# isaac-sim/IsaacGymEnvs

Measured on AMD Instinct MI355X. Metric: env-steps/sec (num_envs x control-steps/sec), random-action rollout, higher is better.
Workload: dtype f32; 1 GPU; Ant num_envs=4096 per GPU (4096 total), VecTask.step() via Python API, actions = 2*torch.rand-1 drawn before every step (README.md:48-51), seed 42+rank; 11000 untimed settle steps (about 0.5 s of back-to-back stepping at the BASELINE size) precede the 5 warm-ups; task=Ant, num_envs_per_gpu=4096, parallelism=env-shard x1, multi_wave=16, fused_sub=1, fused_post=1

## Files before the change

### isaacgymenvs_amd/csrc/core/engine_mw.hpp

```cpp
#pragma once
#include "engine.hpp"

namespace mi {

template <class M>
struct SimMW : Sim<M> {
    using B = Sim<M>;
    using typename B::Ctx;
    using typename B::BodyTmp;
    static constexpr int NB = B::NB, ND = B::ND, NV = B::NV, OFF = B::OFF, NSPH = B::NSPH, NSENS = B::NSENS, NLIM = B::NLIM,
                         NROWG = B::NROWG, NVA = B::NVA, NR = M::NROLE;

    static constexpr int role_of_body(int b) { return M::role_of_limb[M::limb_of_body[b]]; }
    static constexpr int role_of_gi(int gi) { return gi < OFF ? -1 : role_of_body(M::dof_body[gi - OFF]); }
    static constexpr bool trunk_body(int b) { return role_of_body(b) < 0; }
    static constexpr bool trunk_gi(int gi) { return role_of_gi(gi) < 0; }
    template <int R> static constexpr bool owns_body(int b) { return role_of_body(b) == R || (trunk_body(b) && R == M::TRUNK_ROLE); }
    template <int R> static constexpr bool owns_gi(int gi) { return role_of_gi(gi) == R || (trunk_gi(gi) && R == M::TRUNK_ROLE); }
    template <int R> static constexpr bool sees_gi(int gi) { return role_of_gi(gi) == R || trunk_gi(gi); }
    static constexpr int NTB = []() constexpr { int n = 0; for (int b = 0; b < NB; ++b) n += trunk_body(b) ? 1 : 0; return n; }();
    static constexpr int tslot(int b) { int n = 0; for (int k = 0; k < b; ++k) n += trunk_body(k) ? 1 : 0; return n; }
    static constexpr int NVT = []() constexpr { int n = 0; for (int i = 0; i < NV; ++i) n += trunk_gi(i) ? 1 : 0; return n; }();
    static constexpr int tidx(int gi) { int n = 0; for (int k = 0; k < gi; ++k) n += trunk_gi(k) ? 1 : 0; return n; }
    static constexpr int entry_row(int e) {
        for (int i = 0; i < NV; ++i)
            for (int j = 0; j <= i; ++j)
                if (M::midx[i][j] == e) return i;
        return 0;
    }
    static constexpr bool trunk_entry(int e) { return trunk_gi(entry_row(e)); }
    static constexpr int NTE = []() constexpr { int n = 0; for (int e = 0; e < M::NM; ++e) n += trunk_entry(e) ? 1 : 0; return n; }();
    static constexpr int teidx(int e) { int n = 0; for (int k = 0; k < e; ++k) n += trunk_entry(k) ? 1 : 0; return n; }
    static constexpr bool limb_root(int b) { return b > 0 && !trunk_body(b) && trunk_body(M::parent[b]); }
    static constexpr int NLR = []() constexpr { int n = 0; for (int b = 0; b < NB; ++b) n += limb_root(b) ? 1 : 0; return n; }();
    static constexpr int lridx(int b) { int n = 0; for (int k = 0; k < b; ++k) n += limb_root(k) ? 1 : 0; return n; }
    static constexpr int X_LR = B::ROW_SLOTS_STATIC;
    static constexpr int X_DT = X_LR + 16 * NLR;
    static constexpr int X_DY = X_DT + NR * NTE;
    static constexpr int X_DW = X_DY + NR * NVT;
    static constexpr int X_FLG = X_DW + 2 * NR * NVT;
    static constexpr int X_AT = X_FLG + 2 * NR;
    static constexpr int MW_SLOTS = X_AT + NROWG;

    static constexpr int NUNIT = NLIM + NSPH;
    template <int R> static constexpr bool own_unit(int u) {
        if (u < 0 || u >= NUNIT) return false;
        return u < NLIM ? owns_gi<R>(OFF + B::limdof(u)) : owns_body<R>(M::sph_body[u - NLIM]);
    }
    template <int R> static constexpr int next_own(int u) {
        for (int k = u + 1; k < NUNIT; ++k) if (own_unit<R>(k)) return k;
        return NUNIT;
    }
    template <int R> static constexpr int own_pos(int u) { int n = 0; for (int k = 0; k < u; ++k) n += own_unit<R>(k) ? 1 : 0; return n; }

    template <int R, int b, int XLR, int RS>
    MI_HD void trunk_down(const SimParams& P, Ctx& c, BodyTmp (&tb)[NTB], const float* Rp, const float* rp, const float* Vp,
                          const float* Ap, const RowStore<RS> rows) {
        constexpr int ts = tslot(b);
        BodyTmp& t = tb[ts];
        this->template body_down<b>(P, c, Rp, rp, Vp, Ap, t);
        sfor<NB>([&](auto C_) MI_LAMBDA {
            constexpr int ch = C_;
            if constexpr (ch > b) if constexpr (M::parent[ch] == b) {
                if constexpr (trunk_body(ch)) {
                    trunk_down<R, ch, XLR>(P, c, tb, t.Rb, t.rb, t.Vc, t.Ac, rows);
                } else if constexpr (role_of_body(ch) == R) {
                    SpI Ic;
                    float Fc[6];
                    this->template body_pass<ch>(P, c, t.Rb, t.rb, t.Vc, t.Ac, Ic, Fc);
                    constexpr int o = XLR + 16 * lridx(ch);
                    rows(o) = Ic.m;
                    sfor<3>([&](auto K) MI_LAMBDA { rows(o + 1 + K) = Ic.h[K]; });
                    sfor<6>([&](auto K) MI_LAMBDA { rows(o + 4 + K) = Ic.I[K]; rows(o + 10 + K) = Fc[K]; });
                }
            }
        });
    }

    float sens_own[6 * M::NSENSA];
    template <int R, bool KEEP = false, bool SENS = false, int RS, class GND, class BAR>
    MI_HD void substep_role(const SimParams& P, const float* tau, const float h, const RowStore<RS> rows, const Strided lamc,
                            const Strided laml, const Strided sensor, const Strided dof_force, const GND& gnd, const float mu_env,
                            const Strided netf, const int stage, const BAR& bar) {
        static_assert(!M::FIXED, "multi-wave sub-step: free-base models");
        auto G = [&](int row, int cc) MI_LAMBDA -> float& { return rows(row * M::MAXCHAIN + cc); };
        auto Ainv = [&](int row) MI_LAMBDA -> float& { return rows(NROWG * M::MAXCHAIN + row); };
        auto vt = [&](int row) MI_LAMBDA -> float& { return rows(NROWG * M::MAXCHAIN + NROWG + row); };
        auto lam = [&](int row) MI_LAMBDA -> float& { return rows(NROWG * M::MAXCHAIN + 2 * NROWG + row); };
        const float invh = MI_RCP(h);
        float (&root)[13] = this->root;
        float (&q)[M::NDA] = this->q;
        float (&qd)[M::NDA] = this->qd;
#if defined(MI_TIMING)
        unsigned long long* const tstamp = this->tstamp;
#endif
        MI_STAMP(0);
        Ctx c;
        float (&S)[M::NDA][6] = c.S;
        float (&L)[M::NM] = c.L;
        if (stage == 0) {
            sfor<ND>([&](auto D) MI_LAMBDA {
                constexpr int d = D;
                if constexpr (M::dof_limited[d] && owns_gi<R>(OFF + d)) { constexpr int o = B::stage_slot_lim(d); rows(o) = laml(d); }
            });
            sfor<3 * NSPH>([&](auto K) MI_LAMBDA {
                if constexpr (owns_body<R>(M::sph_body[K / 3])) { constexpr int o = B::stage_slot_con(K); rows(o) = lamc(K); }
            });
        }
        BodyTmp tb[NTB];
        static_assert(!B::COMPACT && B::LAM_IN_ROWS, "substep_role: models on the static row store");
        trunk_down<R, 0, X_LR>(P, c, tb, nullptr, nullptr, nullptr, nullptr, rows);
        MI_PHASE();
        float Ldi[NVA], y[NVA], w[NVA], v[NVA];
        v[0] = root[7]; v[1] = root[8]; v[2] = root[9]; v[3] = root[10]; v[4] = root[11]; v[5] = root[12];
        sfor<ND>([&](auto D) MI_LAMBDA { v[OFF + D] = qd[D]; });
        sfor<M::NM>([&](auto E_) MI_LAMBDA { if constexpr (trunk_entry(E_)) L[E_] = 0.f; });
        sfor<NV>([&](auto I) MI_LAMBDA { if constexpr (trunk_gi(I)) y[I] = 0.f; });
        float sc_damp[M::NDA], sc_stiff[M::NDA], sc_arm[M::NDA];
        sfor<ND>([&](auto D) MI_LAMBDA { sc_damp[D] = 1.f; sc_stiff[D] = 1.f; sc_arm[D] = 1.f; });
        if constexpr (B::SCALED) {
            if (this->actor_scale.p != nullptr) {
                sfor<ND>([&](auto D) MI_LAMBDA {
                    if constexpr (sees_gi<R>(OFF + D)) {
                        sc_damp[D] = this->actor_scale(B::AS_DAMP + D); sc_stiff[D] = this->actor_scale(B::AS_STIFF + D); sc_arm[D] = this->actor_scale(B::AS_ARM + D);
                    }
                });
            }
        }
        sfor<ND>([&](auto D) MI_LAMBDA {
            constexpr int d = D, gi = OFF + d;
            if constexpr (role_of_gi(gi) == R) {
                const float K = M::dof_stiffness[d] * sc_stiff[d], Dm = M::dof_damping[d] * sc_damp[d];
                L[M::midx[gi][gi]] += M::dof_armature[d] * sc_arm[d] + h * Dm + h * h * K;
                y[gi] = tau[d] - c.bias[gi] - K * (q[d] - M::dof_springref[d]) - (Dm + h * K) * qd[d];
            }
        });
        auto factor = [&](auto K_) MI_LAMBDA {
            constexpr int k = decltype(K_)::value;
            const float dk2 = fmaxf(L[M::midx[k][k]], 1e-30f);
            const float inv = MI_RSQ(dk2);
            L[M::midx[k][k]] = dk2 * inv;
            Ldi[k] = inv;
            sfor<M::nanc[k]>([&](auto A_) MI_LAMBDA { L[M::midx[k][M::anc[k][A_]]] *= inv; });
            sfor<M::nanc[k]>([&](auto A_) MI_LAMBDA {
                constexpr int i = M::anc[k][A_];
                const float lki = L[M::midx[k][i]];
                L[M::midx[i][i]] -= lki * lki;
                sfor<M::nanc[i]>([&](auto B_) MI_LAMBDA {
                    constexpr int j = M::anc[i][B_];
                    L[M::midx[i][j]] -= lki * L[M::midx[k][j]];
                });
            });
        };
        auto whiten = [&](auto I_) MI_LAMBDA {
            constexpr int i = decltype(I_)::value;
            const float z = y[i] * Ldi[i];
            sfor<M::nanc[i]>([&](auto A_) MI_LAMBDA { y[M::anc[i][A_]] -= L[M::midx[i][M::anc[i][A_]]] * z; });
            float s = L[M::midx[i][i]] * v[i];
            sfor<M::nanc[i]>([&](auto A_) MI_LAMBDA { s += L[M::midx[i][M::anc[i][A_]]] * v[M::anc[i][A_]]; });
            w[i] = s + h * z;
        };
        sfor_rev<NV>([&](auto K_) MI_LAMBDA { if constexpr (role_of_gi(K_) == R) factor(K_); });
        MI_PHASE();
        sfor_rev<NV>([&](auto I_) MI_LAMBDA { if constexpr (role_of_gi(I_) == R) whiten(I_); });
        sfor<M::NM>([&](auto E_) MI_LAMBDA { if constexpr (trunk_entry(E_)) { constexpr int o = X_DT + R * NTE + teidx(E_); rows(o) = L[E_]; } });
        sfor<NV>([&](auto I) MI_LAMBDA { if constexpr (trunk_gi(I)) { constexpr int o = X_DY + R * NVT + tidx(I); rows(o) = y[I]; } });
// ... 220 lines not shown
                        Bf.vt = rit(NROWG * M::MAXCHAIN + NROWG + row0);
                    }
                };
                auto unit_on = [&](auto U_) MI_LAMBDA -> bool {
                    constexpr int u = decltype(U_)::value;
                    if constexpr (u < NLIM) return true;
                    else if constexpr (u < NUNIT) return (sph_active >> (u - NLIM) & 1ull) != 0ull;
                    else return false;
                };
                constexpr int U0 = next_own<R>(-1);
                if constexpr (U0 < NUNIT) load_unit(std::integral_constant<int, U0>{}, ub[0]);
                sfor<NUNIT>([&](auto U_) MI_LAMBDA {
                    constexpr int u = U_;
                    if constexpr (own_unit<R>(u)) {
                        constexpr int pos = own_pos<R>(u), un = next_own<R>(u);
                        UBuf& Bf = ub[pos & 1];
                        if (unit_on(std::integral_constant<int, un>{}))
                            load_unit(std::integral_constant<int, un>{}, ub[(pos + 1) & 1]);
                        MI_PHASE();
                        if (!unit_on(std::integral_constant<int, u>{})) return;
                        if constexpr (u < NLIM) {
                            constexpr int d = B::limdof(u), gi = OFF + d, row = u;
                            float vn = Bf.g[0][0] * wget(std::integral_constant<int, gi>{});
                            sfor<M::nanc[gi]>([&](auto A_) MI_LAMBDA { vn += Bf.g[0][1 + A_] * wget(std::integral_constant<int, M::anc[gi][A_]>{}); });
                            const float lo = Bf.lam[0];
                            const float nl = fmaxf(lo - (vn - Bf.vt) * MI_RCP(Bf.al[0] + om * Bf.at[0]), 0.f);
                            const float dl = nl - lo;
                            lam(row) = nl;
                            actn = (nl > 0.f) ? 1.f : actn;
                            wupd(std::integral_constant<int, gi>{}, Bf.g[0][0] * dl);
                            sfor<M::nanc[gi]>([&](auto A_) MI_LAMBDA { wupd(std::integral_constant<int, M::anc[gi][A_]>{}, Bf.g[0][1 + A_] * dl); });
                        } else {
                            constexpr int s = u - NLIM, b = M::sph_body[s], row0 = NLIM + 3 * s;
                            const float mu = 0.5f * ((mu_env >= 0.f ? mu_env : M::sph_mu[s]) + P.plane_mu);
                            float ainv[3];
                            sfor<3>([&](auto K) MI_LAMBDA { ainv[K] = MI_RCP(Bf.al[K] + om * Bf.at[K]); });
                            float ln;
                            {
                                float vn = 0.f;
                                sfor<M::chain_len[b]>([&](auto C) MI_LAMBDA { vn += Bf.g[0][C] * wget(std::integral_constant<int, M::chain[b][C]>{}); });
                                const float lo = Bf.lam[0];
                                ln = fmaxf(lo - (vn - Bf.vt) * ainv[0], 0.f);
                                const float dl = ln - lo;
                                lam(row0) = ln;
                                actn = (ln > 0.f) ? 1.f : actn;
                                sfor<M::chain_len[b]>([&](auto C) MI_LAMBDA { wupd(std::integral_constant<int, M::chain[b][C]>{}, Bf.g[0][C] * dl); });
                            }
                            float lt[2], vtg[2];
                            sfor<2>([&](auto K) MI_LAMBDA {
                                float vn = 0.f;
                                sfor<M::chain_len[b]>([&](auto C) MI_LAMBDA { vn += Bf.g[1 + K][C] * wget(std::integral_constant<int, M::chain[b][C]>{}); });
                                vtg[K] = vn;
                                lt[K] = Bf.lam[1 + K] - vn * ainv[1 + K];
                            });
                            friction_disc(lt, Bf.lam[1], Bf.lam[2], vtg[0], vtg[1], ainv[1], ainv[2], mu * ln);
                            sfor<2>([&](auto K) MI_LAMBDA {
                                constexpr int row = row0 + 1 + K;
                                const float nl = lt[K], dl = nl - Bf.lam[1 + K];
                                lam(row) = nl;
                                sfor<M::chain_len[b]>([&](auto C) MI_LAMBDA { wupd(std::integral_constant<int, M::chain[b][C]>{}, Bf.g[1 + K][C] * dl); });
                            });
                        }
                    }
                });
                sfor<NV>([&](auto I) MI_LAMBDA { if constexpr (trunk_gi(I)) { constexpr int ti = tidx(I); xout(R * NVT + ti) = (wtl[ti] - w[I]) * iom; } });
                fout(R) = actn;
                bar();
                sfor<NV>([&](auto I) MI_LAMBDA {
                    constexpr int i = I;
                    if constexpr (trunk_gi(i)) { sfor<NR>([&](auto R_) MI_LAMBDA { constexpr int o = R_ * NVT + tidx(i); w[i] += xout(o); }); }
                });
            }
        }
        MI_STAMP(5);
        sfor<NV>([&](auto I_) MI_LAMBDA {
            constexpr int i = I_;
            if constexpr (sees_gi<R>(i)) {
                float s = w[i];
                sfor<M::nanc[i]>([&](auto A_) MI_LAMBDA { s -= L[M::midx[i][M::anc[i][A_]]] * v[M::anc[i][A_]]; });
                v[i] = s * Ldi[i];
            }
        });
        MI_PHASE();
        sfor<ND>([&](auto D) MI_LAMBDA {
            constexpr int d = D;
            if constexpr (owns_gi<R>(OFF + d)) {
                float ll = 0.f;
                if constexpr (M::dof_limited[d]) {
                    constexpr int row = B::limrow(d);
                    const float dl = q[d] - this->template limit_lower<d>(), du = this->template limit_upper<d>() - q[d];
                    ll = (dl < du) ? lam(row) : -lam(row);
                    if constexpr (KEEP) lam(row) = ll;
                }
                laml(d) = ll;
                dof_force(d) = tau[d] - M::dof_stiffness[d] * sc_stiff[d] * (q[d] - M::dof_springref[d]) - M::dof_damping[d] * sc_damp[d] * v[OFF + d] + ll * invh;
            }
        });
        float sens[6 * M::NSENSA];
        sfor<6 * NSENS>([&](auto K) MI_LAMBDA { sens[K] = 0.f; });
        float nf[GND::NETF ? NB : 1][3];
        if constexpr (GND::NETF) sfor<NB>([&](auto B_) MI_LAMBDA { nf[B_][0] = nf[B_][1] = nf[B_][2] = 0.f; });
        sfor<NSPH>([&](auto S_) MI_LAMBDA {
            constexpr int s = S_, b = M::sph_body[s], row0 = NLIM + 3 * s;
            if constexpr (owns_body<R>(b)) {
                if (!(sph_active >> s & 1ull)) {
                    lamc(3 * s) = 0.f; lamc(3 * s + 1) = 0.f; lamc(3 * s + 2) = 0.f;
                    return;
                }
                const float ln = lam(row0), l1 = lam(row0 + 1), l2 = lam(row0 + 2);
                lamc(3 * s) = ln; lamc(3 * s + 1) = l1; lamc(3 * s + 2) = l2;
                float f[3], xc[3];
                if constexpr (GND::HEIGHTFIELD) {
                    float n[3], t1[3], t2[3];
                    n[0] = vt(row0 + 1); n[1] = vt(row0 + 2);
                    n[2] = MI_SQRT(fmaxf(1.f - n[0] * n[0] - n[1] * n[1], 0.f));
                    contact_frame(n, t1, t2);
                    sfor<3>([&](auto K) MI_LAMBDA {
                        f[K] = (n[K] * ln + t1[K] * l1 + t2[K] * l2) * invh;
                        xc[K] = c.xcs[s][K] - M::sph_rad[s] * n[K];
                        nf[b][K] += f[K];
                    });
                } else {
                    f[0] = l1 * invh; f[1] = l2 * invh; f[2] = ln * invh;
                    xc[0] = c.xcs[s][0]; xc[1] = c.xcs[s][1]; xc[2] = c.xcs[s][2] - M::sph_rad[s];
                    if constexpr (GND::NETF) sfor<3>([&](auto K) MI_LAMBDA { nf[b][K] += f[K]; });
                }
                if constexpr (B::sensor_of(b) >= 0) {
                    constexpr int k = B::sensor_of(b);
                    const float arm[3] = {xc[0] - c.rs[k][0], xc[1] - c.rs[k][1], xc[2] - c.rs[k][2]};
                    float tq[3], fl[3], tl[3];
                    cross3(arm, f, tq);
                    matTvec3(c.Rs[k], f, fl); matTvec3(c.Rs[k], tq, tl);
                    sfor<3>([&](auto C) MI_LAMBDA { sens[6 * k + C] += fl[C]; sens[6 * k + 3 + C] += tl[C]; });
                }
            }
        });
        if constexpr (GND::NETF) sfor<NB>([&](auto B_) MI_LAMBDA {
            if constexpr (owns_body<R>(B_)) sfor<3>([&](auto K) MI_LAMBDA { netf(3 * B_ + K) = nf[B_][K]; });
        });
        sfor<NSENS>([&](auto K_) MI_LAMBDA {
            if constexpr (owns_body<R>(M::sens_body[K_])) sfor<6>([&](auto C) MI_LAMBDA {
                sensor(6 * K_ + C) = sens[6 * K_ + C];
                if constexpr (SENS) sens_own[6 * K_ + C] = sens[6 * K_ + C];
            });
        });
        MI_PHASE();
        sfor<ND>([&](auto D) MI_LAMBDA {
            if constexpr (owns_gi<R>(OFF + D)) { qd[D] = v[OFF + D]; q[D] += h * qd[D]; }
        });
        if constexpr (R == M::TRUNK_ROLE) {
#if !defined(MI_NO_VEL_CLAMP)
            {
                const float w2 = v[3] * v[3] + v[4] * v[4] + v[5] * v[5], l2 = v[0] * v[0] + v[1] * v[1] + v[2] * v[2];
                const float sw = (w2 > kMaxAngularVelocity * kMaxAngularVelocity) ? kMaxAngularVelocity * MI_RSQ(w2) : 1.f;
                const float sl = (l2 > kMaxLinearVelocity * kMaxLinearVelocity) ? kMaxLinearVelocity * MI_RSQ(l2) : 1.f;
                v[0] *= sl; v[1] *= sl; v[2] *= sl; v[3] *= sw; v[4] *= sw; v[5] *= sw;
            }
#endif
            sfor<3>([&](auto K) MI_LAMBDA { root[7 + K] = v[K]; root[10 + K] = v[3 + K]; root[K] += h * v[K]; });
            const float om[3] = {v[3], v[4], v[5]};
            const float an = MI_SQRT(dot3(om, om)), th = an * h;
            float dq[4];
            {
                float sn, cs;
                sincosf(0.5f * th, &sn, &cs);
                const bool big = th > 1e-12f;
                const float k = big ? sn * MI_RCP(fmaxf(an, 1e-30f)) : 0.5f * h;
                dq[0] = om[0] * k; dq[1] = om[1] * k; dq[2] = om[2] * k; dq[3] = big ? cs : 1.f;
            }
            float* Q = root + 3;
            const float x = dq[3] * Q[0] + dq[0] * Q[3] + dq[1] * Q[2] - dq[2] * Q[1];
            const float yy = dq[3] * Q[1] - dq[0] * Q[2] + dq[1] * Q[3] + dq[2] * Q[0];
            const float z = dq[3] * Q[2] + dq[0] * Q[1] - dq[1] * Q[0] + dq[2] * Q[3];
            const float ww = dq[3] * Q[3] - dq[0] * Q[0] - dq[1] * Q[1] - dq[2] * Q[2];
            const float n = MI_RSQ(x * x + yy * yy + z * z + ww * ww);
            Q[0] = x * n; Q[1] = yy * n; Q[2] = z * n; Q[3] = ww * n;
        }
        MI_STAMP(6);
    }
};

}
```

### isaacgymenvs_amd/csrc/mw_kernels.hpp

```cpp
#pragma once
#include <cstddef>
#include "step_kernels.hpp"
#include "core/engine_mw.hpp"
#include "tasks/anymal_step.hpp"

namespace mi {

#if defined(MI_TIMING)
__device__ unsigned long long* g_mi_tstamp_mw = nullptr;
#endif
struct DevBarrier {
    __device__ __forceinline__ void operator()() const { __syncthreads(); }
};
template <class M, int E>
constexpr size_t mw_lds_bytes() { return (size_t)SimMW<M>::MW_SLOTS * E * sizeof(float); }
template <class M, class GND, int E, int R>
__device__ __forceinline__ void mw_role(const View& v, const SimParams& P, const ActParams& ap, const float* __restrict__ actions_in,
                                        const int src, const GND& gnd, float* lds_rows, const int e, const int lane, float* post_x = nullptr) {
    using S = SimMW<M>;
    constexpr int ND = M::ND;
    const int N = v.N;
    S sim;
    load_sim(sim, v, e);
    load_actor_scales(sim, v, e);
// ... 30 lines not shown
        typedef __attribute__((address_space(3))) void* lptr_t;
        float* slot0 = lds_rows;
        sfor<ND>([&](auto D) MI_LAMBDA {
            constexpr int d = D;
            if constexpr (M::dof_limited[d] && S::template owns_gi<R>(M::OFF + d)) {
                constexpr int o = Sim<M>::stage_slot_lim(d) * E;
                __builtin_amdgcn_global_load_lds((gptr_t)(v.laml + (size_t)d * N + e), (lptr_t)(slot0 + o), 4, 0, 0);
            }
        });
        sfor<3 * M::NSPH>([&](auto K) MI_LAMBDA {
            if constexpr (S::template owns_body<R>(M::sph_body[K / 3])) {
                constexpr int o = Sim<M>::stage_slot_con(K) * E;
                __builtin_amdgcn_global_load_lds((gptr_t)(v.lamc + (size_t)K * N + e), (lptr_t)(slot0 + o), 4, 0, 0);
            }
        });
    }
    const float h = P.dt / (float)P.substeps;
    const Strided lamc{v.lamc + e, N}, laml{v.laml + e, N}, sensor{v.sensor + e, N}, dof_force{v.dof_force + e, N};
    const Strided netf{GND::NETF ? v.netf + e : nullptr, N};
    const float mu_env = (GND::HEIGHTFIELD || v.friction != nullptr) ? v.friction[e] : -1.f;
    sim.template substep_role<R>(P, tau, h, RowStore<E>{lds_rows + lane}, lamc, laml, sensor, dof_force, gnd, mu_env, netf, true, DevBarrier{});
    sfor<ND>([&](auto K) MI_LAMBDA {
        if constexpr (S::template owns_gi<R>(M::OFF + K)) {
            v.dof[K * N + e] = sim.q[K];
            v.dof[(ND + K) * N + e] = sim.qd[K];
        }
    });
    if constexpr (R == M::TRUNK_ROLE) sfor<13>([&](auto K) MI_LAMBDA { v.root[K * N + e] = sim.root[K]; });
    if (post_x != nullptr) {
        sfor<ND>([&](auto K) MI_LAMBDA {
            if constexpr (S::template owns_gi<R>(M::OFF + K)) { post_x[(13 + K) * E] = sim.q[K]; post_x[(13 + ND + K) * E] = sim.qd[K]; }
        });
        if constexpr (R == M::TRUNK_ROLE) sfor<13>([&](auto K) MI_LAMBDA { post_x[K * E] = sim.root[K]; });
    }
}
template <class M, class GND, int E>
__global__ __launch_bounds__(64 * M::NROLE) void substep_mw_kernel(View v, SimParams P, ActParams ap, const float* __restrict__ actions_in,
                                                                   int src, GND gnd) {
    extern __shared__ float lds_rows[];
    static_assert(M::NROLE == 4, "four roles, one per SIMD of a CU");
    const int lane = threadIdx.x;
    if (lane >= E) return;
    const int e = xcd_env_base<E>(blockIdx.x) + lane;
    if (e >= v.N) return;
    const int role = __builtin_amdgcn_readfirstlane(threadIdx.y);
    switch (role) {
        case 0: mw_role<M, GND, E, 0>(v, P, ap, actions_in, src, gnd, lds_rows, e, lane); break;
        case 1: mw_role<M, GND, E, 1>(v, P, ap, actions_in, src, gnd, lds_rows, e, lane); break;
        case 2: mw_role<M, GND, E, 2>(v, P, ap, actions_in, src, gnd, lds_rows, e, lane); break;
        default: mw_role<M, GND, E, 3>(v, P, ap, actions_in, src, gnd, lds_rows, e, lane); break;
    }
}

template <class GND>
struct MwFusedArgs {
    View v;
    SimParams P;
    ActParams ap;
    const float* actions_in;
    int first, rest, n_sub, tail;
    GND gnd;
    int cmdnorm = 0, cmdnorm_allow_knee = 0;
    float cmdnorm_max_len = 0.f;
};
template <class M, int E>
constexpr size_t mw_fused_lds_bytes() { return (size_t)(SimMW<M>::MW_SLOTS + 13) * E * sizeof(float); }
template <class GND>
struct MwFusedPostArgs {
    MwFusedArgs<GND> f;
    LocoParams tp;
};
template <size_t BEGIN, size_t END>
struct KernargLines {
    static_assert(BEGIN % 4 == 0 && END % 4 == 0 && BEGIN < END, "dword-aligned byte range of the argument struct");
    static constexpr int NL = (int)((END - BEGIN + 63) / 64) + 1;
    uint32_t x[NL];
    __device__ __forceinline__ explicit KernargLines(const void* args) {
        const uint32_t* p = static_cast<const uint32_t*>(args);
        sfor<NL - 1>([&](auto K) MI_LAMBDA { x[K] = p[(BEGIN + 64 * K) / 4]; });
        x[NL - 1] = p[END / 4 - 1];
    }
    __device__ __forceinline__ void drop() const { sfor<NL>([&](auto K) MI_LAMBDA { asm volatile("" ::"s"(x[K])); }); }
};
template <class S, class M, bool HUM, int E, int R, bool BAR_FIRST = false, bool SENS_REG = false>
__device__ __forceinline__ void loco_post_role(const View& v, const LocoParams& tp, S& sim, const float* act, const int e, float* xpost) {
    using T = Loco<M::ND, 6 * M::NSENS, HUM>;
    constexpr int ND = M::ND, NOBS = T::NOBS;
    const int N = v.N;
    if constexpr (BAR_FIRST) __syncthreads();
    const uint32_t genv = (uint32_t)(v.env_offset + e);
    const bool do_reset = v.reset[e] != 0;
    int ep = v.episode[e];
    long long progress = 0, randomize = 0;
    float potentials = 0.f, ep_ret = 0.f;
    if constexpr (R == M::TRUNK_ROLE) { progress = v.progress[e] + 1; potentials = v.potentials[e]; ep_ret = v.ep_ret[e]; randomize = v.randomize[e]; }
    float* ob = v.obs + (size_t)e * NOBS;
    float* oc = v.obs_out + ((size_t)v.ring * N + e) * NOBS;
    const float c = v.clip_obs;
    auto put = [&](const int k, const float x) MI_LAMBDA { ob[k] = x; oc[k] = fminf(fmaxf(x, -c), c); };
    sfor<ND>([&](auto D) MI_LAMBDA {
        constexpr int d = D;
        if constexpr (S::template owns_gi<R>(M::OFF + d)) {
            if (do_reset) {
                T::reset_dof(tp, v.seed, genv, (uint32_t)ep, d, tp.initial_dof_pos[d], tp.dof_lower[d], tp.dof_upper[d], &sim.q[d], &sim.qd[d]);
                v.laml[d * N + e] = 0.f;
            }
            v.dof[d * N + e] = sim.q[d];
            v.dof[(ND + d) * N + e] = sim.qd[d];
            float ps, vs, fs;
            T::obs_dof(tp, sim.q[d], sim.qd[d], HUM ? v.dof_force[d * N + e] : 0.f, tp.dof_lower[d], tp.dof_upper[d], &ps, &vs, &fs);
            const float a_d = (act != nullptr) ? act[d] : v.actions[d * N + e];
            put(T::COL_POS + d, ps);
            put(T::COL_VEL + d, vs);
            if constexpr (HUM) put(T::COL_FORCE + d, fs);
            put(T::COL_ACT + d, a_d);
            typename T::DofSums one;
            T::reward_dof(tp, a_d, ps, vs, tp.gear[d], one);
            xpost[(3 * d + 0) * E] = one.actions; xpost[(3 * d + 1) * E] = one.electricity; xpost[(3 * d + 2) * E] = one.at_limit;
        }
    });
    sfor<M::NSENS>([&](auto K_) MI_LAMBDA {
        constexpr int k = K_;
        if constexpr (S::template owns_body<R>(M::sens_body[k])) {
            float sv[6];
            sfor<6>([&](auto J) MI_LAMBDA {
                if constexpr (SENS_REG) sv[J] = sim.sens_own[6 * k + J]; else sv[J] = v.sensor[(6 * k + J) * N + e];
            });
            sfor<6>([&](auto J) MI_LAMBDA { put(T::COL_SENS + 6 * k + J, sv[J] * tp.contact_force_scale); });
        }
    });
    if (do_reset) sfor<3 * M::NSPH>([&](auto K) MI_LAMBDA { if constexpr (S::template owns_body<R>(M::sph_body[K / 3])) v.lamc[K * N + e] = 0.f; });
    if constexpr (R != M::TRUNK_ROLE) { __syncthreads(); return; }
    float prev_potentials;
    if (do_reset) {
        float init_root[13];
        sfor<13>([&](auto K) MI_LAMBDA { init_root[K] = v.init_root[K * N + e]; sim.root[K] = init_root[K]; });
        const float pp = T::reset_potential(tp, init_root);
        potentials = pp;
        ep += 1;
        progress = 0;
        if constexpr (M::NPG > 0) { if (v.lamp) sfor<3 * M::NPG>([&](auto K) MI_LAMBDA { v.lamp[K * N + e] = 0.f; }); }
    }
    sfor<13>([&](auto K) MI_LAMBDA { v.root[K * N + e] = sim.root[K]; });
    float up_vec[3], heading_vec[3], o12[12];
    T::obs_root(tp, sim.root, tp.targets, potentials, tp.inv_start_rot, tp.basis_vec0, tp.basis_vec1, o12, &potentials, &prev_potentials, up_vec, heading_vec);
    sfor<12>([&](auto K) MI_LAMBDA { put(K, o12[K]); });
    __syncthreads();
    typename T::DofSums part[4];
    sfor<ND>([&](auto D) MI_LAMBDA {
        constexpr int d = D;
        part[d & 3].actions += xpost[(3 * d + 0) * E]; part[d & 3].electricity += xpost[(3 * d + 1) * E]; part[d & 3].at_limit += xpost[(3 * d + 2) * E];
    });
    typename T::DofSums sm;
    sm.actions = (part[0].actions + part[1].actions) + (part[2].actions + part[3].actions);
    sm.electricity = (part[0].electricity + part[1].electricity) + (part[2].electricity + part[3].electricity);
    sm.at_limit = (part[0].at_limit + part[1].at_limit) + (part[2].at_limit + part[3].at_limit);
    float rew;
    long long reset;
    T::reward_total(tp, o12[0], o12[10], o12[11], sm, 0LL, progress, potentials, prev_potentials, &rew, &reset);
    episode_stats<E, true>(v, e, true, rew, reset, progress, ep_ret);
    v.randomize[e] = randomize + 1;
    v.episode[e] = ep;
    v.potentials[e] = potentials;
    v.prev_potentials[e] = prev_potentials;
    sfor<3>([&](auto K) MI_LAMBDA { v.up_vec[K * N + e] = up_vec[K]; v.heading_vec[K * N + e] = heading_vec[K]; });
    v.rew[e] = rew;
    v.reset[e] = reset;
    v.progress[e] = progress;
    v.timeout[e] = (unsigned char)(((float)progress >= tp.max_episode_length - 1.f) && (reset != 0));
}

template <class M, class GND, int E, int R, bool POST = false, bool HUM = false>
__device__ __forceinline__ void mw_role_fused(const MwFusedArgs<GND>& a, float* lds_rows, const int e, const int lane, const LocoParams* tp = nullptr) {
    using S = SimMW<M>;
    constexpr int ND = M::ND;
    const View& v = a.v;
    const ActParams& ap = a.ap;
    const int N = v.N;
    S sim;
#if defined(MI_TIMING)
    unsigned long long* const tstamp = (lane == 0 && g_mi_tstamp_mw != nullptr) ? g_mi_tstamp_mw + ((size_t)blockIdx.x * 4 + R) * 32 : nullptr;
    MI_STAMP(30);
#endif
    load_sim(sim, v, e);
    load_actor_scales(sim, v, e);
    {
        typedef const __attribute__((address_space(1))) void* gptr_t;
        typedef __attribute__((address_space(3))) void* lptr_t;
        float* slot0 = lds_rows;
        sfor<ND>([&](auto D) MI_LAMBDA {
            constexpr int d = D;
            if constexpr (M::dof_limited[d] && S::template owns_gi<R>(M::OFF + d)) {
                constexpr int o = Sim<M>::stage_slot_lim(d) * E;
                __builtin_amdgcn_global_load_lds((gptr_t)(v.laml + (size_t)d * N + e), (lptr_t)(slot0 + o), 4, 0, 0);
            }
        });
        sfor<3 * M::NSPH>([&](auto K) MI_LAMBDA {
            if constexpr (S::template owns_body<R>(M::sph_body[K / 3])) {
                constexpr int o = Sim<M>::stage_slot_con(K) * E;
                __builtin_amdgcn_global_load_lds((gptr_t)(v.lamc + (size_t)K * N + e), (lptr_t)(slot0 + o), 4, 0, 0);
            }
        });
    }
    const float h = a.P.dt / (float)a.P.substeps;
    const Strided lamc{v.lamc + e, N}, laml{v.laml + e, N}, sensor{v.sensor + e, N}, dof_force{v.dof_force + e, N};
    const Strided netf{GND::NETF ? v.netf + e : nullptr, N};
    const float mu_env = (GND::HEIGHTFIELD || v.friction != nullptr) ? v.friction[e] : -1.f;
    float* xroot = lds_rows + (size_t)S::MW_SLOTS * E + lane;
    float tau[M::NDA], act[M::NDA];
    sfor<ND>([&](auto K) MI_LAMBDA { tau[K] = 0.f; act[K] = 0.f; });
    for (int i = 0; i < a.n_sub; ++i) {
        const int src = (i >= a.n_sub - a.tail) ? (i == 0 ? (int)ACT_STORED_TAU : -1) : (i == 0 ? a.first : a.rest);
        if (src == ACT_STORED_TAU) {
            if (i == 0) sfor<ND>([&](auto K) MI_LAMBDA { tau[K] = v.tau[K * N + e]; });
        } else if (src > 0) {
            sfor<ND>([&](auto K) MI_LAMBDA {
                constexpr int k = K;
                constexpr bool mine = S::template owns_gi<R>(M::OFF + k);
                float t = 0.f;
                if (k < ap.nact) {
                    float x;
                    if (src == ACT_FROM_ACTIONS) {
                        x = a.actions_in[(size_t)e * ap.nact + k];
                        x = fminf(fmaxf(x, -ap.clip), ap.clip);
                        if constexpr (mine) v.actions[k * N + e] = x;
                        act[k] = x;
                    } else if (i == 0) {
                        x = v.actions[k * N + e];
                        act[k] = x;
                    } else {
                        x = act[k];
                    }
                    if (ap.mode == 0) {
                        t = x * ap.gear[k] * ap.scale;
                    } else {
                        float qk = sim.q[k], qdk = sim.qd[k];
                        if constexpr (GND::HEIGHTFIELD) {
                            if (i == 0 && v.dof_api != nullptr) { qk = v.dof_api[k * N + e]; qdk = v.dof_api[(ND + k) * N + e]; }
                        }
                        const float u = ap.kp * (ap.scale * x + ap.gear[k] - qk) - ap.kd * qdk;
                        t = fminf(fmaxf(u, -ap.torque_limit), ap.torque_limit);
                    }
                }
                tau[k] = t;
                if constexpr (mine) v.tau[k * N + e] = t;
            });
        }
#if defined(MI_TIMING)
        sim.tstamp = (tstamp != nullptr && i < 3) ? tstamp + 8 * i : nullptr;
#endif
        sim.template substep_role<R, true, POST>(a.P, tau, h, RowStore<E>{lds_rows + lane}, lamc, laml, sensor, dof_force, a.gnd, mu_env, netf,
                                           i == 0 ? 1 : 2, DevBarrier{});
        if constexpr (GND::HEIGHTFIELD) {
            if (i == a.n_sub - a.tail - 1 && v.dof_api != nullptr)
                sfor<ND>([&](auto K) MI_LAMBDA {
                    if constexpr (S::template owns_gi<R>(M::OFF + K)) { v.dof_api[K * N + e] = sim.q[K]; v.dof_api[(ND + K) * N + e] = sim.qd[K]; }
                });
        }
        if (i + 1 < a.n_sub) {
            if constexpr (R == M::TRUNK_ROLE) sfor<13>([&](auto K) MI_LAMBDA { xroot[K * E] = sim.root[K]; });
            __syncthreads();
            if constexpr (R != M::TRUNK_ROLE) sfor<13>([&](auto K) MI_LAMBDA { sim.root[K] = xroot[K * E]; });
        }
    }
    if constexpr (GND::HEIGHTFIELD && !POST) {
        if (a.cmdnorm != 0) {
            __syncthreads();
            if constexpr (R == M::TRUNK_ROLE) {
                bool rs = anymal_netf_norm(v, e, 0) > 1.f;
                if (a.cmdnorm_allow_knee == 0)
                    for (int k = 0; k < 4; ++k) rs = rs || (anymal_netf_norm(v, e, anymal_knee_body(k)) > 1.f);
                if (v.progress[e] + 1 >= (long long)a.cmdnorm_max_len - 1) rs = true;
                float acc = 0.f;
                if (rs) { const float cx = v.commands[e], cy = v.commands[N + e]; acc = cx * cx + cy * cy; }
                acc = wave_sum_live<E>(acc);
                if ((threadIdx.x & 63) == 0 && acc > 0.f) atomicAdd(v.ep_stats + 15, acc);
            }
        }
    }
    if constexpr (POST) {
        static_assert(3 * M::ND <= 16 * S::NLR, "the reward terms fit the (by now dead) tree-pass exchange area");
        loco_post_role<S, M, HUM, E, R, false, true>(v, *tp, sim, act, e, lds_rows + (size_t)S::X_LR * E + lane);
        MI_STAMP(31);
        return;
    }
    sfor<ND>([&](auto K) MI_LAMBDA {
        if constexpr (S::template owns_gi<R>(M::OFF + K)) {
            v.dof[K * N + e] = sim.q[K];
            v.dof[(ND + K) * N + e] = sim.qd[K];
        }
    });
    if constexpr (R == M::TRUNK_ROLE) sfor<13>([&](auto K) MI_LAMBDA { v.root[K * N + e] = sim.root[K]; });
}
template <class M, class GND, int E, bool HUM>
__global__ __launch_bounds__(64 * M::NROLE, E == 8 ? 2 : 1) void substep_mw_fused_post_kernel(MwFusedPostArgs<GND> args_by_value) {
    extern __shared__ float lds_rows[];
    static_assert(M::NROLE == 4, "four roles, one per SIMD of a CU");
#if defined(__HIP_DEVICE_COMPILE__)
    (void)args_by_value;
    const MwFusedPostArgs<GND>& a = *reinterpret_cast<const MwFusedPostArgs<GND>*>(__builtin_amdgcn_kernarg_segment_ptr());
    const int lane = threadIdx.x;
    if (lane >= E) return;
    const KernargLines<offsetof(MwFusedPostArgs<GND>, f.v.potentials), offsetof(MwFusedPostArgs<GND>, f.v.stats) + sizeof(float*)> view_tail(&a);
    const KernargLines<offsetof(MwFusedPostArgs<GND>, tp), sizeof(MwFusedPostArgs<GND>)> task_params(&a);
    const int N = a.f.v.N;
    asm volatile("" ::"s"(N));
    view_tail.drop();
    task_params.drop();
    const int e = xcd_env_base<E>(blockIdx.x) + lane;
    if (e >= N) return;
    const int role = __builtin_amdgcn_readfirstlane(threadIdx.y);
    switch (role) {
        case 0: mw_role_fused<M, GND, E, 0, true, HUM>(a.f, lds_rows, e, lane, &a.tp); break;
        case 1: mw_role_fused<M, GND, E, 1, true, HUM>(a.f, lds_rows, e, lane, &a.tp); break;
        case 2: mw_role_fused<M, GND, E, 2, true, HUM>(a.f, lds_rows, e, lane, &a.tp); break;
        default: mw_role_fused<M, GND, E, 3, true, HUM>(a.f, lds_rows, e, lane, &a.tp); break;
    }
#endif
}
template <class M, class GND, int E>
__global__ __launch_bounds__(64 * M::NROLE) void substep_mw_fused_kernel(MwFusedArgs<GND> args_by_value) {
    extern __shared__ float lds_rows[];
    static_assert(M::NROLE == 4, "four roles, one per SIMD of a CU");
#if defined(__HIP_DEVICE_COMPILE__)
    (void)args_by_value;
    const MwFusedArgs<GND>& a = *reinterpret_cast<const MwFusedArgs<GND>*>(__builtin_amdgcn_kernarg_segment_ptr());
    const int lane = threadIdx.x;
    if (lane >= E) return;
    const int e = xcd_env_base<E>(blockIdx.x) + lane;
    if (e >= a.v.N) return;
    const int role = __builtin_amdgcn_readfirstlane(threadIdx.y);
    switch (role) {
        case 0: mw_role_fused<M, GND, E, 0>(a, lds_rows, e, lane); break;
        case 1: mw_role_fused<M, GND, E, 1>(a, lds_rows, e, lane); break;
        case 2: mw_role_fused<M, GND, E, 2>(a, lds_rows, e, lane); break;
        default: mw_role_fused<M, GND, E, 3>(a, lds_rows, e, lane); break;
    }
#endif
}

template <class M, class GND>
hipError_t launch_substeps_mw(const View& v, const SimParams& P, const ActParams& ap, const float* actions, int n_sub, int first, int rest,
                              hipStream_t s, const GND& gnd, int tail, const MwCmdNormTail* cn) {
    const dim3 block(64, M::NROLE);
    if (v.fused_sub != 0 && n_sub > 1) {
        static unsigned long long fconf16 = 0ull, fconf32 = 0ull;
        constexpr size_t flds16 = mw_fused_lds_bytes<M, 16>(), flds32 = mw_fused_lds_bytes<M, 32>();
        MwFusedArgs<GND> fa{v, P, ap, actions, first, rest, n_sub, tail, gnd};
        if (cn != nullptr) { fa.cmdnorm = 1; fa.cmdnorm_allow_knee = cn->allow_knee_contacts; fa.cmdnorm_max_len = cn->max_episode_length; }
        if (MI_MW_HAS16 && v.mw == 16) {
            auto kern = substep_mw_fused_kernel<M, GND, MI_MW_HAS16 ? 16 : 32>;
            if (hipError_t e = ensure_dynamic_lds((const void*)kern, flds16, &fconf16); e != hipSuccess) return e;
            hipLaunchKernelGGL(kern, dim3(xcd_grid<16>(v.N)), block, flds16, s, fa);
        } else {
            auto kern = substep_mw_fused_kernel<M, GND, 32>;
            if (hipError_t e = ensure_dynamic_lds((const void*)kern, flds32, &fconf32); e != hipSuccess) return e;
            hipLaunchKernelGGL(kern, dim3(xcd_grid<32>(v.N)), block, flds32, s, fa);
        }
        return hipGetLastError();
    }
    static unsigned long long conf16 = 0ull, conf32 = 0ull;
    constexpr size_t lds16 = mw_lds_bytes<M, 16>(), lds32 = mw_lds_bytes<M, 32>();
    auto src_of = [&](int i) { return i >= n_sub - tail ? (int)ACT_STORED_TAU : (i == 0 ? first : rest); };
    if (MI_MW_HAS16 && v.mw == 16) {
        auto kern = substep_mw_kernel<M, GND, MI_MW_HAS16 ? 16 : 32>;
        if (hipError_t e = ensure_dynamic_lds((const void*)kern, lds16, &conf16); e != hipSuccess) return e;
        const dim3 grid(xcd_grid<16>(v.N));
        for (int i = 0; i < n_sub; ++i) hipLaunchKernelGGL(kern, grid, block, lds16, s, v, P, ap, actions, src_of(i), gnd);
    } else {
        auto kern = substep_mw_kernel<M, GND, 32>;
        if (hipError_t e = ensure_dynamic_lds((const void*)kern, lds32, &conf32); e != hipSuccess) return e;
        const dim3 grid(xcd_grid<32>(v.N));
        for (int i = 0; i < n_sub; ++i) hipLaunchKernelGGL(kern, grid, block, lds32, s, v, P, ap, actions, src_of(i), gnd);
    }
    return hipGetLastError();
}

template <class GND>
struct MwPostArgs {
    View v;
    SimParams P;
    ActParams ap;
    const float* actions_in;
    int src;
    GND gnd;
    LocoParams tp;
};
template <class M, class GND, int E, bool HUM>
__global__ __launch_bounds__(64 * M::NROLE) void substep_mw_post_kernel(MwPostArgs<GND> args_by_value) {
    extern __shared__ float lds_rows[];
    static_assert(M::NROLE == 4, "four roles, one per SIMD of a CU");
    static_assert(13 + 2 * M::ND <= 16 * SimMW<M>::NLR, "the new state fits the tree-pass exchange area");
#if defined(__HIP_DEVICE_COMPILE__)
    (void)args_by_value;
    const MwPostArgs<GND>& a = *reinterpret_cast<const MwPostArgs<GND>*>(__builtin_amdgcn_kernarg_segment_ptr());
    const int lane = threadIdx.x;
    if (lane >= E) return;
    const int e = xcd_env_base<E>(blockIdx.x) + lane;
    if (e >= a.v.N) return;
    const int role = __builtin_amdgcn_readfirstlane(threadIdx.y);
    float* post_x = lds_rows + (size_t)SimMW<M>::X_LR * E + lane;
    switch (role) {
        case 0: mw_role<M, GND, E, 0>(a.v, a.P, a.ap, a.actions_in, a.src, a.gnd, lds_rows, e, lane, post_x); break;
        case 1: mw_role<M, GND, E, 1>(a.v, a.P, a.ap, a.actions_in, a.src, a.gnd, lds_rows, e, lane, post_x); break;
        case 2: mw_role<M, GND, E, 2>(a.v, a.P, a.ap, a.actions_in, a.src, a.gnd, lds_rows, e, lane, post_x); break;
        default: mw_role<M, GND, E, 3>(a.v, a.P, a.ap, a.actions_in, a.src, a.gnd, lds_rows, e, lane, post_x); break;
    }
    __syncthreads();
    if (role != M::TRUNK_ROLE) return;
    float root[13], q[M::NDA], qd[M::NDA];
    sfor<13>([&](auto K) MI_LAMBDA { root[K] = post_x[K * E]; });
    sfor<M::ND>([&](auto K) MI_LAMBDA { q[K] = post_x[(13 + K) * E]; qd[K] = post_x[(13 + M::ND + K) * E]; });
    loco_post_env<M, HUM, E, true, false>(a.v, a.tp, e, true, root, q, qd);
// ... 51 lines not shown
```

Measured before the change: 97.87 million env-steps/s.

## Skip non-final substep outputs, split episode stats to another role, prefetch args

Per-substep output writes (limit lambdas, dof forces, contact forces, sensors, net forces) now run only on the last substep of the fused kernel. This removes redundant global stores and contact-force math from intermediate substeps. The episode-statistics reduction moves from the trunk role to a neighbouring role: the trunk publishes eight words through LDS and the other role computes the reward and does a DPP row reduction. Actions, tau and friction loads are hoisted before the LDS setup, and the whole kernarg block is prefetched into scalar registers. The risk is a change in when intermediate outputs are visible, plus extra LDS traffic and a duplicated reward computation.

```diff
diff --git a/isaacgymenvs_amd/csrc/core/engine_mw.hpp b/isaacgymenvs_amd/csrc/core/engine_mw.hpp
--- a/isaacgymenvs_amd/csrc/core/engine_mw.hpp
+++ b/isaacgymenvs_amd/csrc/core/engine_mw.hpp
@@ -78,10 +78,11 @@
     }
 
     float sens_own[6 * M::NSENSA];
-    template <int R, bool KEEP = false, bool SENS = false, int RS, class GND, class BAR>
+    struct AllOutputs { MI_HD constexpr bool operator()() const { return true; } };
+    template <int R, bool KEEP = false, bool SENS = false, int RS, class GND, class BAR, class OUT = AllOutputs>
     MI_HD void substep_role(const SimParams& P, const float* tau, const float h, const RowStore<RS> rows, const Strided lamc,
                             const Strided laml, const Strided sensor, const Strided dof_force, const GND& gnd, const float mu_env,
-                            const Strided netf, const int stage, const BAR& bar) {
+                            const Strided netf, const int stage, const BAR& bar, const OUT& outputs = OUT{}) {
         static_assert(!M::FIXED, "multi-wave sub-step: free-base models");
         auto G = [&](int row, int cc) MI_LAMBDA -> float& { return rows(row * M::MAXCHAIN + cc); };
         auto Ainv = [&](int row) MI_LAMBDA -> float& { return rows(NROWG * M::MAXCHAIN + row); };
@@ -468,6 +469,7 @@
             }
         });
         MI_PHASE();
+        const bool out = outputs();
         sfor<ND>([&](auto D) MI_LAMBDA {
             constexpr int d = D;
             if constexpr (owns_gi<R>(OFF + d)) {
@@ -478,58 +480,62 @@
                     ll = (dl < du) ? lam(row) : -lam(row);
                     if constexpr (KEEP) lam(row) = ll;
                 }
-                laml(d) = ll;
-                dof_force(d) = tau[d] - M::dof_stiffness[d] * sc_stiff[d] * (q[d] - M::dof_springref[d]) - M::dof_damping[d] * sc_damp[d] * v[OFF + d] + ll * invh;
-            }
-        });
-        float sens[6 * M::NSENSA];
-        sfor<6 * NSENS>([&](auto K) MI_LAMBDA { sens[K] = 0.f; });
-        float nf[GND::NETF ? NB : 1][3];
-        if constexpr (GND::NETF) sfor<NB>([&](auto B_) MI_LAMBDA { nf[B_][0] = nf[B_][1] = nf[B_][2] = 0.f; });
-        sfor<NSPH>([&](auto S_) MI_LAMBDA {
-            constexpr int s = S_, b = M::sph_body[s], row0 = NLIM + 3 * s;
-            if constexpr (owns_body<R>(b)) {
-                if (!(sph_active >> s & 1ull)) {
-                    lamc(3 * s) = 0.f; lamc(3 * s + 1) = 0.f; lamc(3 * s + 2) = 0.f;
-                    return;
+                if (out) {
+                    laml(d) = ll;
+                    dof_force(d) = tau[d] - M::dof_stiffness[d] * sc_stiff[d] * (q[d] - M::dof_springref[d]) - M::dof_damping[d] * sc_damp[d] * v[OFF + d] + ll * invh;
                 }
-                const float ln = lam(row0), l1 = lam(row0 + 1), l2 = lam(row0 + 2);
-                lamc(3 * s) = ln; lamc(3 * s + 1) = l1; lamc(3 * s + 2) = l2;
-                float f[3], xc[3];
-                if constexpr (GND::HEIGHTFIELD) {
-                    float n[3], t1[3], t2[3];
-                    n[0] = vt(row0 + 1); n[1] = vt(row0 + 2);
-                    n[2] = MI_SQRT(fmaxf(1.f - n[0] * n[0] - n[1] * n[1], 0.f));
-                    contact_frame(n, t1, t2);
-                    sfor<3>([&](auto K) MI_LAMBDA {
-                        f[K] = (n[K] * ln + t1[K] * l1 + t2[K] * l2) * invh;
-                        xc[K] = c.xcs[s][K] - M::sph_rad[s] * n[K];
-                        nf[b][K] += f[K];
-                    });
-                } else {
-                    f[0] = l1 * invh; f[1] = l2 * invh; f[2] = ln * invh;
-                    xc[0] = c.xcs[s][0]; xc[1] = c.xcs[s][1]; xc[2] = c.xcs[s][2] - M::sph_rad[s];
-                    if constexpr (GND::NETF) sfor<3>([&](auto K) MI_LAMBDA { nf[b][K] += f[K]; });
+            }
+        });
+        if (out) {
+            float sens[6 * M::NSENSA];
+            sfor<6 * NSENS>([&](auto K) MI_LAMBDA { sens[K] = 0.f; });
+            float nf[GND::NETF ? NB : 1][3];
+            if constexpr (GND::NETF) sfor<NB>([&](auto B_) MI_LAMBDA { nf[B_][0] = nf[B_][1] = nf[B_][2] = 0.f; });
+            sfor<NSPH>([&](auto S_) MI_LAMBDA {
+                constexpr int s = S_, b = M::sph_body[s], row0 = NLIM + 3 * s;
+                if constexpr (owns_body<R>(b)) {
+                    if (!(sph_active >> s & 1ull)) {
+                        lamc(3 * s) = 0.f; lamc(3 * s + 1) = 0.f; lamc(3 * s + 2) = 0.f;
+                        return;
+                    }
+                    const float ln = lam(row0), l1 = lam(row0 + 1), l2 = lam(row0 + 2);
+                    lamc(3 * s) = ln; lamc(3 * s + 1) = l1; lamc(3 * s + 2) = l2;
+                    float f[3], xc[3];
+                    if constexpr (GND::HEIGHTFIELD) {
+                        float n[3], t1[3], t2[3];
+                        n[0] = vt(row0 + 1); n[1] = vt(row0 + 2);
+                        n[2] = MI_SQRT(fmaxf(1.f - n[0] * n[0] - n[1] * n[1], 0.f));
+                        contact_frame(n, t1, t2);
+                        sfor<3>([&](auto K) MI_LAMBDA {
+                            f[K] = (n[K] * ln + t1[K] * l1 + t2[K] * l2) * invh;
+                            xc[K] = c.xcs[s][K] - M::sph_rad[s] * n[K];
+                            nf[b][K] += f[K];
+                        });
+                    } else {
+                        f[0] = l1 * invh; f[1] = l2 * invh; f[2] = ln * invh;
+                        xc[0] = c.xcs[s][0]; xc[1] = c.xcs[s][1]; xc[2] = c.xcs[s][2] - M::sph_rad[s];
+                        if constexpr (GND::NETF) sfor<3>([&](auto K) MI_LAMBDA { nf[b][K] += f[K]; });
+                    }
+                    if constexpr (B::sensor_of(b) >= 0) {
+                        constexpr int k = B::sensor_of(b);
+                        const float arm[3] = {xc[0] - c.rs[k][0], xc[1] - c.rs[k][1], xc[2] - c.rs[k][2]};
+                        float tq[3], fl[3], tl[3];
+                        cross3(arm, f, tq);
+                        matTvec3(c.Rs[k], f, fl); matTvec3(c.Rs[k], tq, tl);
+                        sfor<3>([&](auto C) MI_LAMBDA { sens[6 * k + C] += fl[C]; sens[6 * k + 3 + C] += tl[C]; });
+                    }
                 }
-                if constexpr (B::sensor_of(b) >= 0) {
-                    constexpr int k = B::sensor_of(b);
-                    const float arm[3] = {xc[0] - c.rs[k][0], xc[1] - c.rs[k][1], xc[2] - c.rs[k][2]};
-                    float tq[3], fl[3], tl[3];
-                    cross3(arm, f, tq);
-                    matTvec3(c.Rs[k], f, fl); matTvec3(c.Rs[k], tq, tl);
-                    sfor<3>([&](auto C) MI_LAMBDA { sens[6 * k + C] += fl[C]; sens[6 * k + 3 + C] += tl[C]; });
-                }
-            }
-        });
-        if constexpr (GND::NETF) sfor<NB>([&](auto B_) MI_LAMBDA {
-            if constexpr (owns_body<R>(B_)) sfor<3>([&](auto K) MI_LAMBDA { netf(3 * B_ + K) = nf[B_][K]; });
-        });
-        sfor<NSENS>([&](auto K_) MI_LAMBDA {
-            if constexpr (owns_body<R>(M::sens_body[K_])) sfor<6>([&](auto C) MI_LAMBDA {
-                sensor(6 * K_ + C) = sens[6 * K_ + C];
-                if constexpr (SENS) sens_own[6 * K_ + C] = sens[6 * K_ + C];
-            });
-        });
+            });
+            if constexpr (GND::NETF) sfor<NB>([&](auto B_) MI_LAMBDA {
+                if constexpr (owns_body<R>(B_)) sfor<3>([&](auto K) MI_LAMBDA { netf(3 * B_ + K) = nf[B_][K]; });
+            });
+            sfor<NSENS>([&](auto K_) MI_LAMBDA {
+                if constexpr (owns_body<R>(M::sens_body[K_])) sfor<6>([&](auto C) MI_LAMBDA {
+                    sensor(6 * K_ + C) = sens[6 * K_ + C];
+                    if constexpr (SENS) sens_own[6 * K_ + C] = sens[6 * K_ + C];
+                });
+            });
+        }
         MI_PHASE();
         sfor<ND>([&](auto D) MI_LAMBDA {
             if constexpr (owns_gi<R>(OFF + D)) { qd[D] = v[OFF + D]; q[D] += h * qd[D]; }
diff --git a/isaacgymenvs_amd/csrc/mw_kernels.hpp b/isaacgymenvs_amd/csrc/mw_kernels.hpp
--- a/isaacgymenvs_amd/csrc/mw_kernels.hpp
+++ b/isaacgymenvs_amd/csrc/mw_kernels.hpp
@@ -136,10 +136,44 @@
     }
     __device__ __forceinline__ void drop() const { sfor<NL>([&](auto K) MI_LAMBDA { asm volatile("" ::"s"(x[K])); }); }
 };
-template <class S, class M, bool HUM, int E, int R, bool BAR_FIRST = false, bool SENS_REG = false>
+template <int ACTIVE>
+__device__ __forceinline__ float row_sum_live(float v) {
+    static_assert(ACTIVE <= 32, "one or two DPP rows");
+#if defined(__HIP_DEVICE_COMPILE__)
+    auto shl = [](const float x, auto Nn) MI_LAMBDA {
+        constexpr int ctrl = 0x100 + decltype(Nn)::value;
+        return __int_as_float(__builtin_amdgcn_update_dpp(0, __float_as_int(x), ctrl, 0xf, 0xf, true));
+    };
+    v += shl(v, std::integral_constant<int, 8>{});
+    v += shl(v, std::integral_constant<int, 4>{});
+    v += shl(v, std::integral_constant<int, 2>{});
+    v += shl(v, std::integral_constant<int, 1>{});
+    if constexpr (ACTIVE > 16) {
+        const unsigned long long live = __builtin_amdgcn_ballot_w64(true);
+        const float upper = __int_as_float(__builtin_amdgcn_readlane(__float_as_int(v), 16));
+        v += ((live >> 16) & 1ull) ? upper : 0.f;
+    }
+#endif
+    return v;
+}
+template <int E>
+__device__ __forceinline__ void episode_stats_row(const View& v, const int e, const float rew, const long long reset, const long long progress, const float ep_ret) {
+    float ret = ep_ret + rew, fin_ret = 0.f, fin_len = 0.f, fin = 0.f;
+    if (reset != 0) { fin_ret = ret; fin_len = (float)(progress + 1); fin = 1.f; ret = 0.f; }
+    v.ep_ret[e] = ret;
+    fin_ret = row_sum_live<E>(fin_ret); fin_len = row_sum_live<E>(fin_len); fin = row_sum_live<E>(fin);
+    const float r = row_sum_live<E>(rew);
+    if ((threadIdx.x & 63) == 0) {
+        if (fin > 0.f) { stat_add(v.stats + 0, fin_ret); stat_add(v.stats + 1, fin_len); stat_add(v.stats + 2, fin); }
+        stat_add(v.stats + 3, r);
+        if (e == 0) stat_add(v.stats + 4, (float)v.N);
+    }
+}
+template <class S, class M, bool HUM, int E, int R, bool BAR_FIRST = false, bool SENS_REG = false, bool SPLIT = false>
 __device__ __forceinline__ void loco_post_role(const View& v, const LocoParams& tp, S& sim, const float* act, const int e, float* xpost) {
     using T = Loco<M::ND, 6 * M::NSENS, HUM>;
     constexpr int ND = M::ND, NOBS = T::NOBS;
+    constexpr int STAT_ROLE = (M::TRUNK_ROLE + 1) % M::NROLE, XS = 3 * ND;
     const int N = v.N;
     if constexpr (BAR_FIRST) __syncthreads();
     const uint32_t genv = (uint32_t)(v.env_offset + e);
@@ -184,7 +218,32 @@
         }
     });
     if (do_reset) sfor<3 * M::NSPH>([&](auto K) MI_LAMBDA { if constexpr (S::template owns_body<R>(M::sph_body[K / 3])) v.lamc[K * N + e] = 0.f; });
-    if constexpr (R != M::TRUNK_ROLE) { __syncthreads(); return; }
+    auto reward_of = [&](const float o0, const float o10, const float o11, const long long prog, const float pot, const float prev_pot, float* rew,
+                         long long* reset) MI_LAMBDA {
+        typename T::DofSums part[4];
+        sfor<ND>([&](auto D) MI_LAMBDA {
+            constexpr int d = D;
+            part[d & 3].actions += xpost[(3 * d + 0) * E]; part[d & 3].electricity += xpost[(3 * d + 1) * E]; part[d & 3].at_limit += xpost[(3 * d + 2) * E];
+        });
+        typename T::DofSums sm;
+        sm.actions = (part[0].actions + part[1].actions) + (part[2].actions + part[3].actions);
+        sm.electricity = (part[0].electricity + part[1].electricity) + (part[2].electricity + part[3].electricity);
+        sm.at_limit = (part[0].at_limit + part[1].at_limit) + (part[2].at_limit + part[3].at_limit);
+        T::reward_total(tp, o0, o10, o11, sm, 0LL, prog, pot, prev_pot, rew, reset);
+    };
+    if constexpr (R != M::TRUNK_ROLE) {
+        __syncthreads();
+        if constexpr (SPLIT && R == STAT_ROLE) {
+            float pub[8];
+            sfor<8>([&](auto K) MI_LAMBDA { pub[K] = xpost[(XS + K) * E]; });
+            const long long prog = (long long)(((unsigned long long)__float_as_uint(pub[6]) << 32) | (unsigned long long)__float_as_uint(pub[5]));
+            float rew;
+            long long reset;
+            reward_of(pub[0], pub[1], pub[2], prog, pub[3], pub[4], &rew, &reset);
+            episode_stats_row<E>(v, e, rew, reset, prog, pub[7]);
+        }
+        return;
+    }
     float prev_potentials;
     if (do_reset) {
         float init_root[13];
@@ -199,20 +258,18 @@
     float up_vec[3], heading_vec[3], o12[12];
     T::obs_root(tp, sim.root, tp.targets, potentials, tp.inv_start_rot, tp.basis_vec0, tp.basis_vec1, o12, &potentials, &prev_potentials, up_vec, heading_vec);
     sfor<12>([&](auto K) MI_LAMBDA { put(K, o12[K]); });
+    if constexpr (SPLIT) {
+        xpost[(XS + 0) * E] = o12[0]; xpost[(XS + 1) * E] = o12[10]; xpost[(XS + 2) * E] = o12[11];
+        xpost[(XS + 3) * E] = potentials; xpost[(XS + 4) * E] = prev_potentials;
+        xpost[(XS + 5) * E] = __uint_as_float((uint32_t)((unsigned long long)progress & 0xffffffffull));
+        xpost[(XS + 6) * E] = __uint_as_float((uint32_t)((unsigned long long)progress >> 32));
+        xpost[(XS + 7) * E] = ep_ret;
+    }
     __syncthreads();
-    typename T::DofSums part[4];
-    sfor<ND>([&](auto D) MI_LAMBDA {
-        constexpr int d = D;
-        part[d & 3].actions += xpost[(3 * d + 0) * E]; part[d & 3].electricity += xpost[(3 * d + 1) * E]; part[d & 3].at_limit += xpost[(3 * d + 2) * E];
-    });
-    typename T::DofSums sm;
-    sm.actions = (part[0].actions + part[1].actions) + (part[2].actions + part[3].actions);
-    sm.electricity = (part[0].electricity + part[1].electricity) + (part[2].electricity + part[3].electricity);
-    sm.at_limit = (part[0].at_limit + part[1].at_limit) + (part[2].at_limit + part[3].at_limit);
     float rew;
     long long reset;
-    T::reward_total(tp, o12[0], o12[10], o12[11], sm, 0LL, progress, potentials, prev_potentials, &rew, &reset);
-    episode_stats<E, true>(v, e, true, rew, reset, progress, ep_ret);
+    reward_of(o12[0], o12[10], o12[11], progress, potentials, prev_potentials, &rew, &reset);
+    if constexpr (!SPLIT) episode_stats<E, true>(v, e, true, rew, reset, progress, ep_ret);
     v.randomize[e] = randomize + 1;
     v.episode[e] = ep;
     v.potentials[e] = potentials;
@@ -238,6 +295,17 @@
 #endif
     load_sim(sim, v, e);
     load_actor_scales(sim, v, e);
+    float tau[M::NDA], act[M::NDA];
+    sfor<ND>([&](auto K) MI_LAMBDA { tau[K] = 0.f; act[K] = 0.f; });
+    const int src0 = (0 >= a.n_sub - a.tail) ? (int)ACT_STORED_TAU : a.first;
+    if (src0 == ACT_FROM_ACTIONS) {
+        sfor<ND>([&](auto K) MI_LAMBDA { if (K < ap.nact) act[K] = a.actions_in[(size_t)e * ap.nact + K]; });
+    } else if (src0 > 0) {
+        sfor<ND>([&](auto K) MI_LAMBDA { if (K < ap.nact) act[K] = v.actions[K * N + e]; });
+    } else {
+        sfor<ND>([&](auto K) MI_LAMBDA { tau[K] = v.tau[K * N + e]; });
+    }
+    const float mu_env = (GND::HEIGHTFIELD || v.friction != nullptr) ? v.friction[e] : -1.f;
     {
         typedef const __attribute__((address_space(1))) void* gptr_t;
         typedef __attribute__((address_space(3))) void* lptr_t;
@@ -259,15 +327,10 @@
     const float h = a.P.dt / (float)a.P.substeps;
     const Strided lamc{v.lamc + e, N}, laml{v.laml + e, N}, sensor{v.sensor + e, N}, dof_force{v.dof_force + e, N};
     const Strided netf{GND::NETF ? v.netf + e : nullptr, N};
-    const float mu_env = (GND::HEIGHTFIELD || v.friction != nullptr) ? v.friction[e] : -1.f;
     float* xroot = lds_rows + (size_t)S::MW_SLOTS * E + lane;
-    float tau[M::NDA], act[M::NDA];
-    sfor<ND>([&](auto K) MI_LAMBDA { tau[K] = 0.f; act[K] = 0.f; });
     for (int i = 0; i < a.n_sub; ++i) {
         const int src = (i >= a.n_sub - a.tail) ? (i == 0 ? (int)ACT_STORED_TAU : -1) : (i == 0 ? a.first : a.rest);
-        if (src == ACT_STORED_TAU) {
-            if (i == 0) sfor<ND>([&](auto K) MI_LAMBDA { tau[K] = v.tau[K * N + e]; });
-        } else if (src > 0) {
+        if (src > 0) {
             sfor<ND>([&](auto K) MI_LAMBDA {
                 constexpr int k = K;
                 constexpr bool mine = S::template owns_gi<R>(M::OFF + k);
@@ -275,12 +338,9 @@
                 if (k < ap.nact) {
                     float x;
                     if (src == ACT_FROM_ACTIONS) {
-                        x = a.actions_in[(size_t)e * ap.nact + k];
-                        x = fminf(fmaxf(x, -ap.clip), ap.clip);
+                        if (i != 0) act[k] = a.actions_in[(size_t)e * ap.nact + k];
+                        x = fminf(fmaxf(act[k], -ap.clip), ap.clip);
                         if constexpr (mine) v.actions[k * N + e] = x;
-                        act[k] = x;
-                    } else if (i == 0) {
-                        x = v.actions[k * N + e];
                         act[k] = x;
                     } else {
                         x = act[k];
@@ -304,7 +364,7 @@
         sim.tstamp = (tstamp != nullptr && i < 3) ? tstamp + 8 * i : nullptr;
 #endif
         sim.template substep_role<R, true, POST>(a.P, tau, h, RowStore<E>{lds_rows + lane}, lamc, laml, sensor, dof_force, a.gnd, mu_env, netf,
-                                           i == 0 ? 1 : 2, DevBarrier{});
+                                           i == 0 ? 1 : 2, DevBarrier{}, [&]() MI_LAMBDA { return i + 1 == a.n_sub; });
         if constexpr (GND::HEIGHTFIELD) {
             if (i == a.n_sub - a.tail - 1 && v.dof_api != nullptr)
                 sfor<ND>([&](auto K) MI_LAMBDA {
@@ -333,8 +393,8 @@
         }
     }
     if constexpr (POST) {
-        static_assert(3 * M::ND <= 16 * S::NLR, "the reward terms fit the (by now dead) tree-pass exchange area");
-        loco_post_role<S, M, HUM, E, R, false, true>(v, *tp, sim, act, e, lds_rows + (size_t)S::X_LR * E + lane);
+        static_assert(3 * M::ND + 8 <= 16 * S::NLR, "the reward terms and the trunk role's eight words fit the (by now dead) tree-pass exchange area");
+        loco_post_role<S, M, HUM, E, R, false, true, true>(v, *tp, sim, act, e, lds_rows + (size_t)S::X_LR * E + lane);
         MI_STAMP(31);
         return;
     }
@@ -355,12 +415,10 @@
     const MwFusedPostArgs<GND>& a = *reinterpret_cast<const MwFusedPostArgs<GND>*>(__builtin_amdgcn_kernarg_segment_ptr());
     const int lane = threadIdx.x;
     if (lane >= E) return;
-    const KernargLines<offsetof(MwFusedPostArgs<GND>, f.v.potentials), offsetof(MwFusedPostArgs<GND>, f.v.stats) + sizeof(float*)> view_tail(&a);
-    const KernargLines<offsetof(MwFusedPostArgs<GND>, tp), sizeof(MwFusedPostArgs<GND>)> task_params(&a);
+    const KernargLines<0, sizeof(MwFusedPostArgs<GND>)> all_args(&a);
     const int N = a.f.v.N;
     asm volatile("" ::"s"(N));
-    view_tail.drop();
-    task_params.drop();
+    all_args.drop();
     const int e = xcd_env_base<E>(blockIdx.x) + lane;
     if (e >= N) return;
     const int role = __builtin_amdgcn_readfirstlane(threadIdx.y);
@@ -381,8 +439,12 @@
     const MwFusedArgs<GND>& a = *reinterpret_cast<const MwFusedArgs<GND>*>(__builtin_amdgcn_kernarg_segment_ptr());
     const int lane = threadIdx.x;
     if (lane >= E) return;
+    const KernargLines<0, sizeof(MwFusedArgs<GND>)> all_args(&a);
+    const int N = a.v.N;
+    asm volatile("" ::"s"(N));
+    all_args.drop();
     const int e = xcd_env_base<E>(blockIdx.x) + lane;
-    if (e >= a.v.N) return;
+    if (e >= N) return;
     const int role = __builtin_amdgcn_readfirstlane(threadIdx.y);
     switch (role) {
         case 0: mw_role_fused<M, GND, E, 0>(a, lds_rows, e, lane); break;
```

Result: faster. 103.8 million env-steps/s, median of 6 (+6.0%).
